# tuna2134/sbv2-api

Measured on AMD Instinct MI355X. Metric: audio_seconds_per_second, higher is better.
Workload: dtype bf16x3-split (decoder + flow convs: bf16 hi/lo MFMA, f32 accumulate/storage) + f16x3 (DeBERTa GEMMs, flow 1x1: f16 hi + scaled f16 lo per operand, 22 mantissa bits, f32 accumulate) + f32 (text side)

## Files before the change

include/sbv2_hip.h:

```cpp
#ifndef SBV2_HIP_H
#define SBV2_HIP_H

#include <stddef.h>
#include <stdint.h>

#ifdef __cplusplus
extern "C" {
#endif

typedef struct sbv2_bert sbv2_bert;
typedef struct sbv2_vits sbv2_vits;
typedef struct sbv2_pipeline sbv2_pipeline;

const char* sbv2_last_error(void);
int sbv2_device_count(void);

int sbv2_bert_create(const uint8_t* model, size_t model_len, int device, sbv2_bert** out);
void sbv2_bert_destroy(sbv2_bert* h);
int64_t sbv2_bert_hidden(const sbv2_bert* h);
int sbv2_bert_gemm_parts(const sbv2_bert* h);

int sbv2_bert_predict(sbv2_bert* h, const int64_t* token_ids, const int64_t* attention_mask, int64_t S, float* out);
int sbv2_bert_predict_batch(sbv2_bert* h, int64_t n, const int64_t* token_ids, const int64_t* attention_mask,
                            const int64_t* lens, float* out);
// ... 479 lines not shown
                                int64_t N, int poison, float* y, int64_t* stray);
int sbv2_debug_spline_inverse(int device, const float* params, const float* z, const uint8_t* mask, int64_t L, int64_t nbins, float tail, float inv_sqrt_f,
                              int poison, float* z_out, int64_t* stray);
int sbv2_debug_durations(int device, const float* sdp, const float* dp, const uint8_t* mask, int64_t L, float ratio, float length_scale, float* logw,
                         int32_t* dur, int64_t* stray);
int sbv2_debug_durations_rows(int device, const float* sdp, const float* dp, const uint8_t* mask, const int64_t* lens, int nutt, const float* ratio,
                              const float* length_scale, float* logw, int32_t* dur, int64_t* stray);
int sbv2_debug_affine_reverse(int device, const float* z, const float* m, const float* logs, const float* scale, const uint8_t* mask, int64_t L,
                              float* z_out, int64_t* stray);
int sbv2_debug_convflow_pre(int device, const float* z0, const float* w, const float* b, const float* cond, const uint8_t* mask, int64_t C, int64_t L,
                            float* y, int64_t* stray);
int sbv2_debug_noise_fill(int device, const int64_t* lens, int nutt, int kind, const int32_t* seg_utt, uint64_t seed, int stream_id, float scale,
                          int64_t rows, float* y, int64_t* stray);
int sbv2_debug_expand_frames(int device, const float* m_p, const float* logs_p, int64_t C, int64_t Lt, const int32_t* tok_of_frame, const int64_t* lens,
                             int nutt, const int32_t* seg_utt, uint64_t seed, float noise_scale, float* y, int64_t* stray);
int sbv2_debug_noise_fill_rows(int device, const int64_t* lens, int nutt, int kind, const uint64_t* seed, const int32_t* index, int stream_id,
                               const float* scale, int64_t rows, float* y, int64_t* stray);
int sbv2_debug_expand_frames_rows(int device, const float* m_p, const float* logs_p, int64_t C, int64_t Lt, const int32_t* tok_of_frame, const int64_t* lens,
                                  int nutt, const uint64_t* seed, const int32_t* index, const float* noise_scale, float* y, int64_t* stray);
int sbv2_debug_conv_post_tanh(int device, const float* x, const float* w, int64_t C, int64_t k, const int64_t* lens, int nutt, int64_t up, int cl,
                              float* pcm, int64_t* stray);
int sbv2_debug_linear_vec(int device, const float* W, const float* bias, int64_t M, int64_t K, const float* v, int64_t B, float* y);
int sbv2_debug_gather_rows(int device, const float* table, int64_t V, int64_t K, const int32_t* idx, int64_t B, float* y);
int sbv2_debug_text_embed(int device, const int32_t* phones, const int32_t* tones, const int32_t* langs, const int64_t* lens, int nutt, const float* emb,
                          int64_t nph, const float* tone_emb, int64_t ntone, const float* lang_emb, int64_t nlang, const float* bertproj,
                          const float* styleproj, float scale, int64_t H, float* y, int64_t* stray);
int sbv2_debug_add_segvec(int device, const float* x, const float* vec, int64_t C, const int64_t* lens, int nutt, int kind, int64_t div,
                          const uint8_t* tok_mask, int use_mask, int cl, float* y, int64_t* stray);
int sbv2_debug_plane_op(int device, int op, const float* x, int64_t C, int64_t L, const int32_t* map, int64_t a, int64_t b, float* y, uint8_t* mask_out,
                        int64_t* stray);
int sbv2_debug_stream_windows(int device, const float* z, int64_t C, int64_t L, const int32_t* table, int64_t W, int64_t nwin, const float* cond_vecs,
                              int64_t n_rows, int64_t cond_dim, float* z_out, uint8_t* mask_out, float* cond_out);
int sbv2_debug_copy_segments(int device, const float* src, int64_t nsrc, const int64_t* table, int nseg, float* dst, int64_t ndst);

#ifdef __cplusplus
}
#endif
#endif
```

sbv2-api_amd/_lib.py:

```python
import ctypes as C
import os

_HERE = os.path.dirname(os.path.abspath(__file__))
LIB_PATH = os.path.join(_HERE, "libsbv2_hip.so")

i64p = C.POINTER(C.c_int64)
f32p = C.POINTER(C.c_float)


class Sbv2Batch(C.Structure):
    _fields_ = [
        ("n", C.c_int64), ("t_lens", i64p), ("x_tst", i64p), ("tones", i64p), ("lang_ids", i64p), ("sids", i64p),
        ("style_vectors", f32p), ("bert", f32p),
        ("sdp_ratio", C.c_float), ("length_scale", C.c_float), ("noise_scale", C.c_float), ("noise_scale_w", C.c_float),
        ("noise_seed", C.c_uint64), ("forced_durations", i64p),
    ]


class Sbv2PcmFormat(C.Structure):
    _fields_ = [("sample_rate", C.c_int32), ("encoding", C.c_int32), ("normalize", C.c_int32), ("reserved", C.c_int32)]


class Sbv2Loudness(C.Structure):
    _fields_ = [("target_lufs", C.c_double), ("true_peak_max_dbtp", C.c_double)]
# ... 338 lines not shown
                                         i64p]),
    "sbv2_debug_gemm_bfs_ex": (C.c_int, [C.c_int, f32p, f32p, f32p, f32p, C.c_int64, C.c_int64, C.c_int64, C.c_int, C.c_int, C.c_int, C.c_int64, C.c_void_p,
                                         C.c_int64, C.c_float, C.c_float, C.c_int64, C.c_int64, C.c_int, f32p, f32p, f32p, i64p]),
    "sbv2_debug_linear_tokmajor": (C.c_int, [C.c_int, f32p, f32p, f32p, C.c_int64, C.c_int64, C.c_int64, C.c_int64, f32p, i64p]),
    "sbv2_debug_vits_attention": (C.c_int, [C.c_int, f32p, f32p, f32p, f32p, f32p, i64p, C.c_int, C.c_int64, C.c_int64, C.c_int64, C.c_int, C.c_int,
                                            C.c_int, f32p, i64p]),
    "sbv2_debug_deberta_attention": (C.c_int, [C.c_int, f32p, f32p, f32p, f32p, f32p, i64p, C.c_int, C.c_int64, C.c_int64, C.c_int64, C.c_int64,
                                               C.c_void_p, C.c_int64, C.c_int, C.c_int, f32p, i64p]),
    "sbv2_debug_layout": (C.c_int, [i64p, C.c_int, C.c_int, C.POINTER(C.c_int32), i64p]),
    "sbv2_debug_layernorm": (C.c_int, [C.c_int, f32p, f32p, f32p, C.c_float, C.c_int, f32p, C.c_void_p, f32p, f32p, C.c_int64, C.c_int64, C.c_int64, C.c_int,
                                       C.c_int, C.c_int, f32p, f32p, i64p]),
    "sbv2_debug_deberta_embed_ln": (C.c_int, [C.c_int, C.POINTER(C.c_int32), f32p, C.c_int64, C.c_int64, f32p, f32p, C.c_float, C.c_int64, C.c_int, f32p,
                                              i64p]),
    "sbv2_debug_spline_inverse": (C.c_int, [C.c_int, f32p, f32p, C.c_void_p, C.c_int64, C.c_int64, C.c_float, C.c_float, C.c_int, f32p, i64p]),
    "sbv2_debug_durations": (C.c_int, [C.c_int, f32p, f32p, C.c_void_p, C.c_int64, C.c_float, C.c_float, f32p, C.POINTER(C.c_int32), i64p]),
    "sbv2_debug_durations_rows": (C.c_int, [C.c_int, f32p, f32p, C.c_void_p, i64p, C.c_int, f32p, f32p, f32p, C.POINTER(C.c_int32), i64p]),
    "sbv2_debug_affine_reverse": (C.c_int, [C.c_int, f32p, f32p, f32p, f32p, C.c_void_p, C.c_int64, f32p, i64p]),
    "sbv2_debug_convflow_pre": (C.c_int, [C.c_int, f32p, f32p, f32p, f32p, C.c_void_p, C.c_int64, C.c_int64, f32p, i64p]),
    "sbv2_debug_noise_fill": (C.c_int, [C.c_int, i64p, C.c_int, C.c_int, C.POINTER(C.c_int32), C.c_uint64, C.c_int, C.c_float, C.c_int64, f32p, i64p]),
    "sbv2_debug_expand_frames": (C.c_int, [C.c_int, f32p, f32p, C.c_int64, C.c_int64, C.POINTER(C.c_int32), i64p, C.c_int, C.POINTER(C.c_int32), C.c_uint64,
                                           C.c_float, f32p, i64p]),
    "sbv2_debug_noise_fill_rows": (C.c_int, [C.c_int, i64p, C.c_int, C.c_int, C.POINTER(C.c_uint64), C.POINTER(C.c_int32), C.c_int, f32p, C.c_int64, f32p,
                                             i64p]),
    "sbv2_debug_expand_frames_rows": (C.c_int, [C.c_int, f32p, f32p, C.c_int64, C.c_int64, C.POINTER(C.c_int32), i64p, C.c_int, C.POINTER(C.c_uint64),
                                                C.POINTER(C.c_int32), f32p, f32p, i64p]),
    "sbv2_debug_conv_post_tanh": (C.c_int, [C.c_int, f32p, f32p, C.c_int64, C.c_int64, i64p, C.c_int, C.c_int64, C.c_int, f32p, i64p]),
    "sbv2_debug_linear_vec": (C.c_int, [C.c_int, f32p, f32p, C.c_int64, C.c_int64, f32p, C.c_int64, f32p]),
    "sbv2_debug_gather_rows": (C.c_int, [C.c_int, f32p, C.c_int64, C.c_int64, C.POINTER(C.c_int32), C.c_int64, f32p]),
    "sbv2_debug_text_embed": (C.c_int, [C.c_int, C.POINTER(C.c_int32), C.POINTER(C.c_int32), C.POINTER(C.c_int32), i64p, C.c_int, f32p, C.c_int64, f32p,
                                        C.c_int64, f32p, C.c_int64, f32p, f32p, C.c_float, C.c_int64, f32p, i64p]),
    "sbv2_debug_add_segvec": (C.c_int, [C.c_int, f32p, f32p, C.c_int64, i64p, C.c_int, C.c_int, C.c_int64, C.c_void_p, C.c_int, C.c_int, f32p, i64p]),
    "sbv2_debug_plane_op": (C.c_int, [C.c_int, C.c_int, f32p, C.c_int64, C.c_int64, C.POINTER(C.c_int32), C.c_int64, C.c_int64, f32p, C.c_void_p, i64p]),
    "sbv2_debug_copy_segments": (C.c_int, [C.c_int, f32p, C.c_int64, i64p, C.c_int, f32p, C.c_int64]),
}

_lib = None


class Sbv2Error(RuntimeError):
    """Mirror of sbv2_core::error::Error::OtherError (crates/sbv2_core/src/error.rs:29-30)."""


def lib():
    global _lib
    if _lib is None:
        if not os.path.exists(LIB_PATH):
            raise Sbv2Error(f"{LIB_PATH} is missing: build it with __graft_entry__.build() (there is no CPU fallback)")
        l = C.CDLL(LIB_PATH)
        for name, (res, args) in SYMBOLS.items():
            fn = getattr(l, name)
            fn.restype = res
            fn.argtypes = args
        _lib = l
    return _lib


def check(rc):
    if rc != 0:
        raise Sbv2Error(lib().sbv2_last_error().decode(errors="replace"))
```

sbv2-api_amd/csrc/common.h:

```cpp
#pragma once
#include <hip/hip_runtime.h>

#include <atomic>

#include <cstdint>
#include <cstdio>
#include <map>
#include <memory>
#include <stdexcept>
#include <exception>
#include <string>
#include <vector>

namespace sbv2 {

void set_last_error(const std::string& msg);

struct Error : std::runtime_error {
    using std::runtime_error::runtime_error;
};

#define HIP_CHECK(expr)                                                                          \
    do {                                                                                         \
        hipError_t _e = (expr);                                                                  \
// ... 417 lines not shown
    int shift0 = 0, shift_step = 1;
    float* Y = nullptr;
    int ldy = 0;
    float* Ykm = nullptr;
    int ldykm = 0;
    const float* Rkm = nullptr;
    int ldrkm = 0;
    SplitClPlanes Ys;
    float ys_slope = 1.0f;
    const float* bias = nullptr;
    const float* R = nullptr;
    int ldr = 0;
    float beta = 1.0f;
    int accumulate = 0;
    const unsigned char* mask = nullptr;
    int mask_shift = -1;
    int out_stride = 1, phase_rows = 0;
    int phase_off[kMaxPhases] = {0};
    int phase_group = 1;
    int phase_tap0[kMaxPhases] = {0};
    double prof_flops = 0.0;
};
int64_t clx_grid_workgroups(const ConvClxParams& p);
bool conv_clx_usable(const ConvClxParams& p);
int set_clx(int on);
int set_upx(int on);
int set_resbranch(int on);
int set_respair_clx(int on);
bool ksplit_enabled();
int set_ksplit(int on);
bool clx_wanted(int64_t tiles, int64_t min_tiles);
void launch_conv_clx(const ConvClxParams& p, hipStream_t stream);

struct ResPairParams {
    const float* X = nullptr;
    float* Y = nullptr;
    const void* W1 = nullptr;
    const void* W2 = nullptr;
    const void* W1p = nullptr;
    const void* W2p = nullptr;
    const void* W1x = nullptr;
    const void* W2x = nullptr;
    const float* b1 = nullptr;
    const float* b2 = nullptr;
    int C = 0, N = 0, k = 1, dil = 1, split = 1, f16 = 0;
    float slope = 0.1f, beta = 1.0f;
    int accumulate = 0;
    const unsigned char* mask = nullptr;
    int mask_div = 1;
    int mask_shift = -1;
    int alias_x2 = 1;
    int nt_store = 0;
};
void launch_respair_cl(const ResPairParams& p, hipStream_t stream);
bool respair_clx_usable(const ResPairParams& p);
void launch_respair_clx(const ResPairParams& p, hipStream_t stream);
bool respair_x16_usable(const ResPairParams& p);
void launch_respair_x16(const ResPairParams& p, hipStream_t stream);
enum class BranchKernel { resbranch, clx_steps, respair_x16, respair_clx, respair_cl, conv_cl_steps };
BranchKernel respair_default(const ResPairParams& p);
void launch_respair(const ResPairParams& p, BranchKernel kernel, hipStream_t stream);

constexpr int kResBranchSteps = 3;
constexpr int kResBranchMargin = 6;
struct ResBranchParams {
    const float* X = nullptr;
// ... 17 lines not shown
```

sbv2-api_amd/csrc/models.h:

```cpp
#pragma once
#include "common.h"
#include "flac_encode.h"
#include "limiter.h"
#include "marks.h"
#include "ops.h"
#include "pcm_format.h"
#include "stream_output.h"

#include <memory>

namespace sbv2 {

struct ClConv {
    void* w = nullptr;
    void* wxp = nullptr;
    void* wx = nullptr;
    void* wp = nullptr;
    float* bias = nullptr;
    int M = 0, K = 0, k = 1, nmt = 0, tm = 1, parts = 0;
};

struct PackedConv {
    float* w = nullptr;
    float* bias = nullptr;
// ... 67 lines not shown
    float* upload(const float* host, size_t n);
    float* tensor(const std::string& name);
    float* tensor(const std::string& name, std::initializer_list<int64_t> dims);
    void expect(const PackedConv& c, const std::string& prefix, int cout, int cin, int k) const;
    PackedConv conv(const std::string& prefix, bool bias = true);
    PackedConv conv_cat(const std::vector<std::string>& prefixes);
    PackedConv linear(const std::string& prefix);
    PackedUpsample upsample(const std::string& prefix, int stride, int padding);
    size_t bytes() const { return bytes_; }
    const Blob& blob() const { return blob_; }

  private:
    const Blob& blob_;
    int cl_parts_ = 0, bfs_parts_ = 0;
    std::vector<void*> allocs_;
    size_t bytes_ = 0;
};

void conv_plain(const PackedConv& w, Plane x, Plane y, int dil, int pad_l, const unsigned char* mask, int mask_div, hipStream_t s,
                int act = ACT_NONE, float pre_slope = 1.0f, const Plane* res = nullptr, float alpha = 1.0f, float beta = 1.0f,
                int accumulate = 0);
void conv_bfs(const PackedConv& w, const SplitPlanes& xs, const Plane* y, const SplitPlanes* ys, const unsigned char* mask, int mask_div,
              hipStream_t s, int act = ACT_NONE, const Plane* res = nullptr, float alpha = 1.0f, float beta = 1.0f, int y_rows = -1, int ys_row0 = 0,
              const BfsSplitK* sk = nullptr);
bool conv_km_to_cl(const PackedConv& w, Plane x, float* y, int ldy, int dil, int pad_l, const unsigned char* mask, int mask_div,
                   hipStream_t s);
bool conv_cl_to_km(const PackedConv& w, const float* x, int ldx, Plane y, int dil, int pad_l, const unsigned char* mask, int mask_div,
                   hipStream_t s, float pre_slope, const Plane* res);
void linear_tokmajor(const PackedConv& w, Plane x, float* y, int ldy, hipStream_t s);

int default_bert_bfs_parts();
bool flash_parts_enabled();
int set_flash_parts(int on);
bool sdp_all();
int set_sdp_all(int on);

constexpr int kTextGap = 16;
constexpr int kFrameGap = 4;
struct AttnPlan {
    int ng = 0, maxT = 0, lds = 0;
    AttnGroup* d_ag = nullptr;
    GemmGroup* d_st = nullptr;
    GemmGroup* d_pv = nullptr;
    float* S = nullptr;
    float* PW = nullptr;
    double flops = 0;
};
AttnPlan make_attn_plan(const SegLayout& lay, int H, int heads, int ld, int window, Arena& ar, hipStream_t stream, bool scores);
void grouped_gemm(const float* A, int lda, const float* B, int ldb, float* C, int ldc, const GemmGroup* grp, int ng, int maxM, int maxN,
                  float alpha, double flops, hipStream_t s);
struct FlashChoice {
    bool kv_parts = false;
    int pipelined = 1;
};
FlashChoice flash_choice(const AttnPlan& pl, int SP, bool split_attn, int dk);

enum DebertaAttnMode {
    kDbAuto = -1,
    kDbUnfused = 0,
    kDbShort = 1,
    kDbMid = 2,
    kDbLong = 3,
    kDbNoLong = 4,
};
struct DebertaAttnPlan {
    int span = 0, maxT = 0, lds = 0;
// ... 314 lines not shown
```

sbv2-api_amd/csrc/vits.cpp:

```cpp
#include <algorithm>
#include <cmath>
#include <cstring>
#include <memory>

#include <atomic>
#include "models.h"

namespace sbv2 {

static std::atomic<int> g_flash_parts{1};
bool flash_parts_enabled() { return g_flash_parts.load(std::memory_order_relaxed) != 0; }
static int flash_parts_mode() { return g_flash_parts.load(std::memory_order_relaxed); }
int set_flash_parts(int on) { return g_flash_parts.exchange(on); }

static std::atomic<int> g_sdp_all{0};
bool sdp_all() { return g_sdp_all.load(std::memory_order_relaxed) != 0; }
int set_sdp_all(int on) { return g_sdp_all.exchange(on != 0); }

AttnPlan make_attn_plan(const SegLayout& lay, int H, int heads, int ld, int window, Arena& ar, hipStream_t stream, bool scores) {
    AttnPlan pl;
    const int dk = H / heads;
    pl.ng = lay.n * heads;
    pl.maxT = lay.max_len();
    pl.lds = round_up(pl.maxT, 4);
    std::vector<AttnGroup> ag(pl.ng);
    std::vector<GemmGroup> st(pl.ng), pv(pl.ng);
    int64_t s_off = 0, w_off = 0;
    for (int u = 0; u < lay.n; ++u)
        for (int h = 0; h < heads; ++h) {
            const int gi = u * heads + h;
            const int T = lay.len[u];
            AttnGroup& a = ag[gi];
            a.qk_off = (int64_t)h * dk * ld + lay.start[u];
            a.s_off = s_off;
            a.aux_off = w_off;
            a.aux2_off = 0;
            a.T = T;
            a.lds = pl.lds;
            a.col0 = lay.start[u];
            a.head = h;
            st[gi] = GemmGroup{a.qk_off, a.qk_off, s_off, 0, T, T, dk, T};
            pv[gi] = GemmGroup{(int64_t)lay.start[u] * H + h * dk, s_off, a.qk_off, 0, dk, T, T, T};
            pl.flops += 2.0 * (double)T * T * dk;
            s_off += (int64_t)T * pl.lds;
            w_off += (int64_t)(2 * window + 1) * pl.lds;
        }
// ... 280 lines not shown
    if (it == traces_.end()) return false;
    const TraceEntry& t = it->second;
    if (utt < 0 || utt >= t.lay->n) return false;
    HIP_CHECK(hipSetDevice(device_));
    rows = t.p.C;
    cols = t.lay->len[utt] * t.div;
    out.resize((size_t)rows * cols);
    HIP_CHECK(hipStreamSynchronize(stream_));
    HIP_CHECK(hipMemcpy2D(out.data(), sizeof(float) * cols, t.p.p + (size_t)t.lay->start[utt] * t.div, sizeof(float) * t.p.ld,
                          sizeof(float) * cols, rows, hipMemcpyDeviceToHost));
    return true;
}

void VitsModel::run_encoder(const Encoder& e, Plane x, const SegLayout& lay, const float* spk_vec, Arena& ar) {
    const int H = x.C, heads = cfg_.heads, dk = H / heads, N = lay.L;
    const Arena::Mark mk = ar.mark();
    static const bool fused = !(getenv("SBV2_ATTN") && std::string(getenv("SBV2_ATTN")) == "unfused");
    static const bool attn_f32 = getenv("SBV2_ATTN") && std::string(getenv("SBV2_ATTN")) == "f32";
    const bool split_attn = !attn_f32 && e.layers[0].ffn1.cl.parts == 2 && (H / heads) % 16 == 0;
    const AttnPlan pl = make_attn_plan(lay, H, heads, x.ld, cfg_.window, ar, stream_, !fused);
    Plane QKV = ar.plane(3 * H, N);
    Plane Q = QKV.rows(0, H), K = QKV.rows(H, H), ctx = ar.plane(H, N), Y = ar.plane(H, N);
    SBV2_REQUIRE(Q.ld == x.ld, "plane pitch mismatch");
    Plane F = ar.plane(e.layers[0].ffn1.cout, N);
    constexpr bool cl_ffn = true;
    const PackedConv& f1 = e.layers[0].ffn1;
    const PackedConv& f2 = e.layers[0].ffn2;
    float* Fcl = (cl_ffn && f1.cl.parts && f2.cl.parts && f1.k >= 3 && f2.k >= 3 && (f1.cout & 15) == 0) ? ar.array<float>((size_t)N * f1.cout) : nullptr;
    float* VT = fused ? nullptr : ar.array<float>((size_t)N * H);
    Plane Vp = QKV.rows(2 * H, H);
    fill_zero(ctx.p, sizeof(float) * (size_t)H * ctx.ld, stream_);
    const float qscale = 1.0f / std::sqrt((float)dk);
    const int SP = !fused ? 0 : (e.layers[0].attn.qkv.bfs.f16 ? kPartsF16x3 : e.layers[0].attn.qkv.bfs.parts);
    SplitPlanes Xs, Cs, QKVs;
    if (SP) {
        Xs = alloc_split(ar, SP, H, N);
        Cs = alloc_split(ar, SP, H, N);
        split_planes(x, Xs, stream_);
    }
    const FlashChoice fc = flash_choice(pl, SP, split_attn, dk);
    const bool kv_parts = fc.kv_parts;
    if (kv_parts) QKVs = alloc_split(ar, 2, 3 * H, N);
    const bool clx_ffn = Fcl && f1.cl.parts == 2 && f2.cl.parts == 2 && f1.k == 5 && f2.k == 5 && (H & 63) == 0 && (f1.cout & 63) == 0 &&
                         clx_wanted((int64_t)(N / 256) * (H / 64), 192);
    SplitClPlanes XsC, FsC;
    if (clx_ffn) {
        XsC = make_split_cl(ar.alloc(split_cl_bytes(H, N)), H, N, stream_);
        FsC = make_split_cl(ar.alloc(split_cl_bytes(f1.cout, N)), f1.cout, N, stream_);
    }
    for (size_t i = 0; i < e.layers.size(); ++i) {
        const EncLayer& L = e.layers[i];
        if ((int)i == cfg_.cond_layer_idx && spk_vec) {
            add_segvec(x, spk_vec, H, lay.d_seg_of, 1, lay.d_mask, stream_);
            if (SP) split_planes(x, Xs, stream_);
        }
        if (fused) {
            if (SP && kv_parts) conv_bfs(L.attn.qkv, Xs, &QKV, &QKVs, nullptr, 1, stream_, ACT_NONE, nullptr, 1.0f, 1.0f, H, H);
            else if (SP) conv_bfs(L.attn.qkv, Xs, &QKV, nullptr, nullptr, 1, stream_);
            else conv_plain(L.attn.qkv, x, QKV, 1, 0, nullptr, 1, stream_);
            if (kv_parts)
                vits_flash_attention_parts(pl.d_ag, pl.ng, pl.maxT, Q.p, Q.ld, QKVs, H, 2 * H, ctx.p, ctx.ld, dk, L.attn.erk, L.attn.erv, cfg_.window,
                                           qscale, stream_, fc.pipelined);
            else
                vits_flash_attention(pl.d_ag, pl.ng, pl.maxT, Q.p, K.p, Vp.p, Q.ld, ctx.p, ctx.ld, dk, L.attn.erk, L.attn.erv, cfg_.window, qscale,
                                     split_attn, stream_);
        } else {
            conv_plain(L.attn.q, x, Q, 1, 0, nullptr, 1, stream_);
            conv_plain(L.attn.k, x, K, 1, 0, nullptr, 1, stream_);
            linear_tokmajor(L.attn.v, x, VT, H, stream_);
            grouped_gemm(K.p, K.ld, Q.p, Q.ld, pl.S, pl.lds, pl.d_st, pl.ng, pl.maxT, pl.maxT, qscale, pl.flops, stream_);
            vits_softmax(pl.d_ag, pl.ng, pl.maxT, pl.S, Q.p, Q.ld, dk, L.attn.erk, cfg_.window, qscale, pl.PW, stream_);
            grouped_gemm(VT, H, pl.S, pl.lds, ctx.p, ctx.ld, pl.d_pv, pl.ng, dk, pl.maxT, 1.0f, pl.flops, stream_);
            vits_relv_add(pl.d_ag, pl.ng, pl.maxT, ctx.p, ctx.ld, dk, L.attn.erv, cfg_.window, pl.PW, stream_);
        }
        if (SP) {
            split_planes(ctx, Cs, stream_);
            conv_bfs(L.attn.o, Cs, &Y, nullptr, nullptr, 1, stream_, ACT_NONE, &x);
        } else {
            conv_plain(L.attn.o, ctx, Y, 1, 0, nullptr, 1, stream_, ACT_NONE, 1.0f, &x);
        }
        layernorm_ch(Y, x, L.n1g, L.n1b, 1e-5f, ACT_NONE, nullptr, 0, lay.d_mask, stream_);
        const int k = L.ffn1.k;
        const int Fc = L.ffn1.cout;
        if (clx_ffn) {
            split_cl_km(x, 1.0f, XsC, stream_);
            ConvClxParams p1;
            p1.X = XsC;
            p1.W = L.ffn1.cl.wx;
            p1.nmt = L.ffn1.cl.nmt;
            p1.M = Fc;
            p1.N = N;
            p1.K = H;
            p1.ntaps = k;
            p1.shift0 = -(k - 1) / 2;
            p1.shift_step = 1;
            p1.Ys = FsC;
            p1.ys_slope = 0.0f;
            p1.bias = L.ffn1.bias;
            p1.mask = lay.d_mask;
            p1.mask_shift = 0;
            launch_conv_clx(p1, stream_);
            ConvClxParams p2;
            p2.X = FsC;
            p2.W = L.ffn2.cl.wx;
            p2.nmt = L.ffn2.cl.nmt;
            p2.M = H;
            p2.N = N;
            p2.K = Fc;
            p2.ntaps = k;
            p2.shift0 = -(k - 1) / 2;
            p2.shift_step = 1;
            p2.Ykm = Y.p;
            p2.ldykm = Y.ld;
            p2.Rkm = x.p;
            p2.ldrkm = x.ld;
            p2.bias = L.ffn2.bias;
            p2.mask = lay.d_mask;
            p2.mask_shift = 0;
            launch_conv_clx(p2, stream_);
        } else if (Fcl && conv_km_to_cl(L.ffn1, x, Fcl, Fc, 1, (k - 1) / 2, lay.d_mask, 1, stream_)) {
            SBV2_REQUIRE(conv_cl_to_km(L.ffn2, Fcl, Fc, Y, 1, (k - 1) / 2, lay.d_mask, 1, stream_, 0.0f, &x), "FFN: conv_2 has no matrix-core path");
        } else {
            conv_plain(L.ffn1, x, F, 1, (k - 1) / 2, lay.d_mask, 1, stream_, ACT_RELU);
            conv_plain(L.ffn2, F, Y, 1, (k - 1) / 2, lay.d_mask, 1, stream_, ACT_NONE, 1.0f, &x);
        }
        layernorm_ch(Y, x, L.n2g, L.n2b, 1e-5f, ACT_NONE, nullptr, 0, lay.d_mask, stream_, (SP && i + 1 < e.layers.size()) ? &Xs : nullptr);
    }
    ar.rewind(mk);
}

void VitsModel::run_dds(const DDS& d, Plane x, const SegLayout& lay, Arena& ar, int shape_L) {
    const Arena::Mark mk = ar.mark();
    Plane a = ar.plane(x.C, x.L), b = ar.plane(x.C, x.L);
    int dil = 1;
    for (size_t i = 0; i < d.pw.size(); ++i) {
        dds_dw_ln_gelu(x, a, d.sep_w[i], d.sep_b[i], dil, d.n1g[i], d.n1b[i], lay.d_mask, stream_, shape_L);
        conv_plain(d.pw[i], a, b, 1, 0, nullptr, 1, stream_);
        layernorm_ch(b, x, d.n2g[i], d.n2b[i], 1e-5f, ACT_GELU, x.p, x.ld, lay.d_mask, stream_, nullptr, shape_L);
        dil *= cfg_.sdp_kernel;
    }
    ar.rewind(mk);
}

void VitsModel::run_decoder(Arena& ar, Plane z, const SegLayout& fl, const float* cond_vec) {
    const int n = fl.n;
    const int Lf = fl.L;
    Plane cur = ar.plane(cfg_.up_initial, Lf);
    conv_plain(dec_pre_, z, cur, 1, dec_pre_.k / 2, fl.d_mask, 1, stream_);
    add_segvec(cur, cond_vec, cfg_.up_initial, fl.d_seg_of, 1, fl.d_mask, stream_);
    trace("dec_pre", cur, fl, 1);
    int U = 1;
    const int nk = (int)cfg_.res_kernels.size();
    for (size_t si = 0; si < stages_.size(); ++si) {
        const Stage& st = stages_[si];
        U *= st.rate;
        const int Lo = Lf * U;
        Plane XS = ar.plane(st.ch, Lo);
        const Arena::Mark mk = ar.mark();
        Plane XU = ar.plane(st.ch, Lo), T1 = ar.plane(st.ch, Lo), YA = ar.plane(st.ch, Lo), YB = ar.plane(st.ch, Lo);
// ... 672 lines not shown
```

Before: 4833.

## Fuse flow encoder attention-out projection with layernorm and FFN tail with next QKV

```diff
diff --git a/include/sbv2_hip.h b/include/sbv2_hip.h
--- a/include/sbv2_hip.h
+++ b/include/sbv2_hip.h
@@ -535,6 +535,14 @@
 int sbv2_debug_stream_windows(int device, const float* z, int64_t C, int64_t L, const int32_t* table, int64_t W, int64_t nwin, const float* cond_vecs,
                               int64_t n_rows, int64_t cond_dim, float* z_out, uint8_t* mask_out, float* cond_out);
 int sbv2_debug_copy_segments(int device, const float* src, int64_t nsrc, const int64_t* table, int nseg, float* dst, int64_t ndst);
+int sbv2_debug_set_flow_cols(int mode);
+int sbv2_debug_set_flow_cols_block(int nct);
+int sbv2_debug_flow_attn_tail(int device, const float* ctx, const float* x, const float* w, const float* bias, const float* gamma, const float* beta, float eps,
+                              const uint8_t* mask, int64_t N, int64_t ld, int want_parts, int64_t iters, float* x_out, uint16_t* parts, float* ms,
+                              int64_t* stray);
+int sbv2_debug_flow_ffn_tail_qkv(int device, const float* y, const float* gamma, const float* beta, float eps, const uint8_t* mask, const float* spk, int64_t nseg,
+                                 const int32_t* seg_of, const float* w, const float* bias, int64_t N, int64_t ld, int kv_parts, int64_t iters, float* x_out,
+                                 float* qkv, uint16_t* kv, float* ms, int64_t* stray);
 
 #ifdef __cplusplus
 }
diff --git a/sbv2-api_amd/_lib.py b/sbv2-api_amd/_lib.py
--- a/sbv2-api_amd/_lib.py
+++ b/sbv2-api_amd/_lib.py
@@ -394,6 +394,12 @@
     "sbv2_debug_add_segvec": (C.c_int, [C.c_int, f32p, f32p, C.c_int64, i64p, C.c_int, C.c_int, C.c_int64, C.c_void_p, C.c_int, C.c_int, f32p, i64p]),
     "sbv2_debug_plane_op": (C.c_int, [C.c_int, C.c_int, f32p, C.c_int64, C.c_int64, C.POINTER(C.c_int32), C.c_int64, C.c_int64, f32p, C.c_void_p, i64p]),
     "sbv2_debug_copy_segments": (C.c_int, [C.c_int, f32p, C.c_int64, i64p, C.c_int, f32p, C.c_int64]),
+    "sbv2_debug_set_flow_cols": (C.c_int, [C.c_int]),
+    "sbv2_debug_set_flow_cols_block": (C.c_int, [C.c_int]),
+    "sbv2_debug_flow_attn_tail": (C.c_int, [C.c_int, f32p, f32p, f32p, f32p, f32p, f32p, C.c_float, C.c_void_p, C.c_int64, C.c_int64, C.c_int, C.c_int64,
+                                            f32p, C.c_void_p, f32p, i64p]),
+    "sbv2_debug_flow_ffn_tail_qkv": (C.c_int, [C.c_int, f32p, f32p, f32p, C.c_float, C.c_void_p, f32p, C.c_int64, C.POINTER(C.c_int32), f32p, f32p, C.c_int64,
+                                               C.c_int64, C.c_int, C.c_int64, f32p, f32p, C.c_void_p, f32p, i64p]),
 }
 
 _lib = None
diff --git a/sbv2-api_amd/csrc/common.h b/sbv2-api_amd/csrc/common.h
--- a/sbv2-api_amd/csrc/common.h
+++ b/sbv2-api_amd/csrc/common.h
@@ -473,6 +473,48 @@
 bool clx_wanted(int64_t tiles, int64_t min_tiles);
 void launch_conv_clx(const ConvClxParams& p, hipStream_t stream);
 
+constexpr int kFlowColsH = 192;
+struct FlowAttnTailParams {
+    const float* ctx = nullptr;
+    int ldc = 0;
+    float* x = nullptr;
+    int ldx = 0;
+    const void* w = nullptr;
+    int nmt = 0;
+    const float* bias = nullptr;
+    const float* gamma = nullptr;
+    const float* beta = nullptr;
+    float eps = 1e-5f;
+    const unsigned char* mask = nullptr;
+    int N = 0;
+    SplitClPlanes xs;
+    unsigned long long* sat = nullptr;
+};
+struct FlowFfnTailParams {
+    const float* Y = nullptr;
+    int ldy = 0;
+    float* x = nullptr;
+    int ldx = 0;
+    const float* gamma = nullptr;
+    const float* beta = nullptr;
+    float eps = 1e-5f;
+    const unsigned char* mask = nullptr;
+    const float* spk = nullptr;
+    int spk_ld = 0;
+    const int* seg_of = nullptr;
+    const void* w = nullptr;
+    int nmt = 0;
+    const float* bias = nullptr;
+    float* qkv = nullptr;
+    int ldq = 0;
+    SplitPlanes kv;
+    int N = 0;
+    unsigned long long* sat = nullptr;
+};
+void launch_flow_attn_tail(const FlowAttnTailParams& p, hipStream_t stream);
+void launch_flow_ffn_tail_qkv(const FlowFfnTailParams& p, hipStream_t stream);
+int set_flow_cols_block(int nct);
+
 struct ResPairParams {
     const float* X = nullptr;
     float* Y = nullptr;
diff --git a/sbv2-api_amd/csrc/flow_cols.hip b/sbv2-api_amd/csrc/flow_cols.hip
--- /dev/null
+++ b/sbv2-api_amd/csrc/flow_cols.hip
@@ -0,0 +1,387 @@
+#include <atomic>
+
+#include "common.h"
+#include "device_prims.h"
+
+namespace sbv2 {
+
+namespace {
+
+constexpr int kH = kFlowColsH;
+constexpr int kNCH = kH / 16;
+constexpr int kBStr = 2 * kH + 16;
+constexpr int kFStr = kH + 4;
+static_assert(kH == 192, "three 32-row tiles per wave, two waves per column tile");
+
+template <int NCT>
+struct Shape {
+    static constexpr int NB = 32 * NCT, NQ = NB / 4, T = 128 * NCT, NW = 2 * NCT;
+    static constexpr int BPART = NB * kBStr;
+    static constexpr int IMG = 2 * BPART;
+    static constexpr int RED = 2 * 2 * NB * (int)sizeof(float);
+    static constexpr int TILES = NW * 32 * 36 * (int)sizeof(float);
+    static_assert(NB * kFStr * (int)sizeof(float) <= IMG, "the result image fits the operand image");
+    static_assert(2 * 16 * NQ * 16 <= TILES, "the partial sums fit the transpose tiles");
+};
+
+__device__ __forceinline__ void split_f16(float v, _Float16& h, _Float16& l, unsigned& nclamp, bool count) {
+    const float c = (v != v || fabsf(v) == __builtin_inff()) ? v : fminf(fmaxf(v, -65504.f), 65504.f);
+    nclamp += (count && c != v && v == v) ? 1u : 0u;
+    h = (_Float16)c;
+    l = (_Float16)((c - (float)h) * kF16LoScale);
+}
+
+template <int NCT>
+__device__ __forceinline__ void stage_operand(char* img, const f32x4v (&v)[3][4], int cq, int kq0, int n0, int N, unsigned& nclamp) {
+    using S = Shape<NCT>;
+#pragma unroll
+    for (int i = 0; i < 3; ++i)
+#pragma unroll
+        for (int e = 0; e < 4; ++e) {
+            f16x4 h, l;
+            const bool count = n0 + 4 * cq + e < N;
+#pragma unroll
+            for (int j = 0; j < 4; ++j) {
+                _Float16 hh, ll;
+                split_f16(v[i][j][e], hh, ll, nclamp, count);
+                h[j] = hh;
+                l[j] = ll;
+            }
+            char* dst = img + (4 * cq + e) * kBStr + (kq0 + 16 * i) * 8;
+            *reinterpret_cast<f16x4*>(dst) = h;
+            *reinterpret_cast<f16x4*>(dst + S::BPART) = l;
+        }
+}
+
+template <int NCT>
+__device__ __forceinline__ void product(const char* img, const void* w, int nmt, int mt0, int ct, int lane, f32x16 (&acc)[3], f32x16 (&accx)[3]) {
+    using S = Shape<NCT>;
+    const char* wl = static_cast<const char*>(w) + lane * 16;
+    const char* bl = img + (ct * 32 + (lane & 31)) * kBStr + (lane >> 5) * 16;
+    constexpr int kAhead = 3, NBUF = kAhead + 1;
+    f16x8 a[NBUF][3][2];
+    auto load = [&](int c, f16x8 (&f)[3][2]) {
+#pragma unroll
+        for (int i = 0; i < 3; ++i)
+#pragma unroll
+            for (int pp = 0; pp < 2; ++pp) f[i][pp] = *reinterpret_cast<const f16x8*>(wl + ((int64_t)(c * nmt + mt0 + i) * 2 + pp) * 1024);
+    };
+#pragma unroll
+    for (int i = 0; i < 3; ++i)
+#pragma unroll
+        for (int r = 0; r < 16; ++r) acc[i][r] = accx[i][r] = 0.f;
+#pragma unroll
+    for (int c = 0; c < kAhead; ++c) load(c, a[c]);
+#pragma unroll
+    for (int c = 0; c < kNCH; ++c) {
+        if (c + kAhead < kNCH) load(c + kAhead, a[(c + kAhead) % NBUF]);
+        __builtin_amdgcn_sched_barrier(0);
+        const f16x8 bh = *reinterpret_cast<const f16x8*>(bl + c * 32), bo = *reinterpret_cast<const f16x8*>(bl + S::BPART + c * 32);
+        const f16x8(&f)[3][2] = a[c % NBUF];
+#pragma unroll
+        for (int i = 0; i < 3; ++i) accx[i] = mfma32(f[i][1], bh, accx[i]);
+#pragma unroll
+        for (int i = 0; i < 3; ++i) accx[i] = mfma32(f[i][0], bo, accx[i]);
+#pragma unroll
+        for (int i = 0; i < 3; ++i) acc[i] = mfma32(f[i][0], bh, acc[i]);
+    }
+}
+
+template <int NCT>
+__global__ __launch_bounds__(128 * NCT) __attribute__((amdgpu_waves_per_eu(2))) void k_flow_attn_tail(const FlowAttnTailParams p) {
+    using S = Shape<NCT>;
+    extern __shared__ __attribute__((aligned(16))) char smem[];
+    char* img = smem;
+    float* fimg = reinterpret_cast<float*>(smem);
+    float* red = reinterpret_cast<float*>(smem + S::IMG);
+    const int tid = threadIdx.x, lane = tid & 63, wave = tid >> 6;
+    const int n0 = blockIdx.x * S::NB, N = p.N;
+    const int cq = tid % S::NQ, kq0 = tid / S::NQ;
+    const int nq = n0 + 4 * cq, nql = nq < N ? nq : 0;
+    unsigned nclamp = 0;
+    {
+        f32x4v v[3][4];
+#pragma unroll
+        for (int i = 0; i < 3; ++i)
+#pragma unroll
+            for (int j = 0; j < 4; ++j) v[i][j] = *reinterpret_cast<const f32x4v*>(p.ctx + (int64_t)(4 * (kq0 + 16 * i) + j) * p.ldc + nql);
+        stage_operand<NCT>(img, v, cq, kq0, n0, N, nclamp);
+    }
+    if (p.sat && nclamp) atomicAdd(p.sat, (unsigned long long)nclamp);
+    __syncthreads();
+    const int mh = wave & 1, ct = wave >> 1, lh = lane >> 5;
+    const int col = ct * 32 + (lane & 31), n = n0 + col, nl = n < N ? n : 0;
+    f32x16 acc[3], accx[3];
+    product<NCT>(img, p.w, p.nmt, 3 * mh, ct, lane, acc, accx);
+    float s = 0.f;
+#pragma unroll
+    for (int i = 0; i < 3; ++i)
+#pragma unroll
+        for (int r = 0; r < 16; ++r) {
+            const int m = (3 * mh + i) * 32 + (r & 3) + 8 * (r >> 2) + 4 * lh;
+            float y = acc[i][r] + accx[i][r] * (1.0f / kF16LoScale) + p.bias[m];
+            y += p.x[(int64_t)m * p.ldx + nl];
+            acc[i][r] = y;
+            s += y;
+        }
+    s += __shfl_xor(s, 32);
+    if (lh == 0) red[mh * S::NB + col] = s;
+    __syncthreads();
+    const float mean = (red[col] + red[S::NB + col]) / (float)kH;
+    float q = 0.f;
+#pragma unroll
+    for (int i = 0; i < 3; ++i)
+#pragma unroll
+        for (int r = 0; r < 16; ++r) {
+            const float d = acc[i][r] - mean;
+            q += d * d;
+        }
+    q += __shfl_xor(q, 32);
+    if (lh == 0) red[(2 + mh) * S::NB + col] = q;
+    __syncthreads();
+    const float var = red[2 * S::NB + col] + red[3 * S::NB + col];
+    const float rstd = 1.0f / sqrtf(var / kH + p.eps);
+    const bool keep = n < N && (!p.mask || p.mask[nl]);
+#pragma unroll
+    for (int i = 0; i < 3; ++i)
+#pragma unroll
+        for (int g = 0; g < 4; ++g) {
+            const int m = (3 * mh + i) * 32 + 8 * g + 4 * lh;
+            const f32x4v ga = *reinterpret_cast<const f32x4v*>(p.gamma + m), be = *reinterpret_cast<const f32x4v*>(p.beta + m);
+            f32x4v y;
+#pragma unroll
+            for (int e = 0; e < 4; ++e) {
+                const float t = (acc[i][4 * g + e] - mean) * rstd * ga[e] + be[e];
+                y[e] = keep ? t : 0.f;
+            }
+            *reinterpret_cast<f32x4v*>(fimg + col * kFStr + m) = y;
+        }
+    __syncthreads();
+#pragma unroll
+    for (int i = 0; i < 3; ++i) {
+        const int k4 = 4 * (kq0 + 16 * i);
+        f32x4v r[4];
+#pragma unroll
+        for (int e = 0; e < 4; ++e) r[e] = *reinterpret_cast<const f32x4v*>(fimg + (4 * cq + e) * kFStr + k4);
+#pragma unroll
+        for (int j = 0; j < 4; ++j) {
+            float* dst = p.x + (int64_t)(k4 + j) * p.ldx + nq;
+            if (nq + 4 <= N) {
+                *reinterpret_cast<f32x4v*>(dst) = f32x4v{r[0][j], r[1][j], r[2][j], r[3][j]};
+            } else {
+#pragma unroll
+                for (int e = 0; e < 4; ++e)
+                    if (nq + e < N) dst[e] = r[e][j];
+            }
+        }
+    }
+    if (p.xs.p) {
+        const int64_t plane = (int64_t)(p.xs.front + p.xs.N + p.xs.back) * 32;
+#pragma unroll
+        for (int i = 0; i < 3; ++i) {
+            const int u = tid + S::T * i, pc = u % S::NB, ch = u / S::NB;
+            if (n0 + pc >= N) continue;
+            bf16x8 h[2], l[2];
+#pragma unroll
+            for (int g = 0; g < 4; ++g) {
+                const f32x4v v = *reinterpret_cast<const f32x4v*>(fimg + pc * kFStr + ch * 16 + 4 * g);
+#pragma unroll
+                for (int e = 0; e < 4; ++e) {
+                    const __bf16 hh = (__bf16)v[e];
+                    h[g >> 1][(g & 1) * 4 + e] = hh;
+                    l[g >> 1][(g & 1) * 4 + e] = (__bf16)(v[e] - (float)hh);
+                }
+            }
+            char* dst = static_cast<char*>(p.xs.p) + ((int64_t)ch * 2) * plane + ((int64_t)p.xs.front + n0 + pc) * 32;
+            *reinterpret_cast<bf16x8*>(dst) = h[0];
+            *reinterpret_cast<bf16x8*>(dst + 16) = h[1];
+            *reinterpret_cast<bf16x8*>(dst + plane) = l[0];
+            *reinterpret_cast<bf16x8*>(dst + plane + 16) = l[1];
+        }
+    }
+}
+
+template <int NCT>
+__global__ __launch_bounds__(128 * NCT) __attribute__((amdgpu_waves_per_eu(2))) void k_flow_ffn_tail_qkv(const FlowFfnTailParams p) {
+    using S = Shape<NCT>;
+    typedef f32x4v red_t[S::NQ];
+    extern __shared__ __attribute__((aligned(16))) char smem[];
+    char* img = smem;
+    const int tid = threadIdx.x, lane = tid & 63, wave = tid >> 6;
+    const int n0 = blockIdx.x * S::NB, N = p.N;
+    const int cq = tid % S::NQ, kq0 = tid / S::NQ;
+    const int nq = n0 + 4 * cq, nql = nq < N ? nq : 0;
+    unsigned nclamp = 0;
+    {
+        red_t* red = reinterpret_cast<red_t*>(smem + S::IMG);
+        f32x4v v[3][4];
+        f32x4v s = {0.f, 0.f, 0.f, 0.f};
+#pragma unroll
+        for (int i = 0; i < 3; ++i)
+#pragma unroll
+            for (int j = 0; j < 4; ++j) {
+                v[i][j] = *reinterpret_cast<const f32x4v*>(p.Y + (int64_t)(4 * (kq0 + 16 * i) + j) * p.ldy + nql);
+                s += v[i][j];
+            }
+        auto reduce = [&](red_t* r, f32x4v part) {
+            r[kq0][cq] = part;
+            __syncthreads();
+            f32x4v t = r[0][cq];
+#pragma unroll
+            for (int g = 1; g < 16; ++g) t += r[g][cq];
+            return t;
+        };
+        const f32x4v mean = reduce(red, s) / (float)kH;
+        f32x4v q = {0.f, 0.f, 0.f, 0.f};
+#pragma unroll
+        for (int i = 0; i < 3; ++i)
+#pragma unroll
+            for (int j = 0; j < 4; ++j) {
+                const f32x4v d = v[i][j] - mean;
+                q += d * d;
+            }
+        const f32x4v var = reduce(red + 16, q);
+        f32x4v rstd;
+        bool keep[4];
+        int sg[4];
+#pragma unroll
+        for (int e = 0; e < 4; ++e) {
+            rstd[e] = 1.0f / sqrtf(var[e] / kH + p.eps);
+            const int ne = nq + e < N ? nq + e : 0;
+            keep[e] = nq + e < N && (!p.mask || p.mask[ne]);
+            sg[e] = p.spk ? p.seg_of[ne] : -1;
+        }
+#pragma unroll
+        for (int i = 0; i < 3; ++i) {
+            const int k4 = 4 * (kq0 + 16 * i);
+            const f32x4v ga = *reinterpret_cast<const f32x4v*>(p.gamma + k4), be = *reinterpret_cast<const f32x4v*>(p.beta + k4);
+#pragma unroll
+            for (int j = 0; j < 4; ++j) {
+                f32x4v y;
+#pragma unroll
+                for (int e = 0; e < 4; ++e) {
+                    const float t = (v[i][j][e] - mean[e]) * rstd[e] * ga[j] + be[j];
+                    y[e] = keep[e] ? t : 0.f;
+                    if (p.spk) y[e] = (sg[e] >= 0 && keep[e]) ? y[e] + p.spk[(int64_t)sg[e] * p.spk_ld + k4 + j] : 0.f;
+                }
+                v[i][j] = y;
+                float* dst = p.x + (int64_t)(k4 + j) * p.ldx + nq;
+                if (nq + 4 <= N) {
+                    *reinterpret_cast<f32x4v*>(dst) = y;
+                } else {
+#pragma unroll
+                    for (int e = 0; e < 4; ++e)
+                        if (nq + e < N) dst[e] = y[e];
+                }
+            }
+        }
+        stage_operand<NCT>(img, v, cq, kq0, n0, N, nclamp);
+    }
+    if (p.sat && nclamp) atomicAdd(p.sat, (unsigned long long)nclamp);
+    __syncthreads();
+    const int mh = wave & 1, ct = wave >> 1, lh = lane >> 5, lcol = lane & 31;
+    const int lrow = lane >> 3, c4 = (lane & 7) * 4;
+    float* tile = reinterpret_cast<float*>(smem + S::IMG) + wave * (32 * 36);
+    const int nc = n0 + ct * 32 + c4;
+#pragma unroll 1
+    for (int pass = 0; pass < 3; ++pass) {
+        f32x16 acc[3], accx[3];
+        const int mt0 = 6 * pass + 3 * mh;
+        product<NCT>(img, p.w, p.nmt, mt0, ct, lane, acc, accx);
+        const bool parts = p.kv.p && pass > 0;
+#pragma unroll
+        for (int i = 0; i < 3; ++i) {
+#pragma unroll
+            for (int r = 0; r < 16; ++r) tile[((r & 3) + 8 * (r >> 2) + 4 * lh) * 36 + lcol] = acc[i][r] + accx[i][r] * (1.0f / kF16LoScale);
+#pragma unroll
+            for (int ps = 0; ps < 4; ++ps) {
+                const f32x4v av = *reinterpret_cast<const f32x4v*>(tile + (ps * 8 + lrow) * 36 + c4);
+                const int m = (mt0 + i) * 32 + ps * 8 + lrow;
+                const float b = p.bias[m];
+                float v[4];
+#pragma unroll
+                for (int e = 0; e < 4; ++e) v[e] = av[e] + b;
+                if (nc >= N) continue;
+                if (!parts) {
+                    float* dst = p.qkv + (int64_t)m * p.ldq + nc;
+                    if (nc + 4 <= N) {
+                        *reinterpret_cast<f32x4v*>(dst) = f32x4v{v[0], v[1], v[2], v[3]};
+                    } else {
+#pragma unroll
+                        for (int e = 0; e < 4; ++e)
+                            if (nc + e < N) dst[e] = v[e];
+                    }
+                } else {
+                    bf16x4 h, l;
+#pragma unroll
+                    for (int e = 0; e < 4; ++e) {
+                        h[e] = (__bf16)v[e];
+                        l[e] = (__bf16)(v[e] - (float)h[e]);
+                    }
+                    __bf16* dst = static_cast<__bf16*>(p.kv.p) + (int64_t)m * p.kv.ld + nc;
+                    if (nc + 4 <= N) {
+                        *reinterpret_cast<bf16x4*>(dst) = h;
+                        *reinterpret_cast<bf16x4*>(dst + p.kv.pstride) = l;
+                    } else {
+#pragma unroll
+                        for (int e = 0; e < 4; ++e)
+                            if (nc + e < N) {
+                                dst[e] = h[e];
+                                dst[p.kv.pstride + e] = l[e];
+                            }
+                    }
+                }
+            }
+        }
+    }
+}
+
+std::atomic<int> g_block{2};
+
+template <class P>
+void check_common(const P& p, int rows, const char* what) {
+    SBV2_REQUIRE(p.w && p.bias && p.gamma && p.beta && p.N >= 1 && p.nmt * 32 >= rows, what);
+}
+
+template <int NCT, class K, class P>
+void launch_cfg(K kern, const P& p, size_t lds, hipStream_t stream, std::atomic<uint64_t>& done) {
+    allow_full_lds(reinterpret_cast<const void*>(kern), done);
+    hipLaunchKernelGGL(kern, dim3((p.N + 32 * NCT - 1) / (32 * NCT)), dim3(128 * NCT), lds, stream, p);
+    HIP_CHECK(hipGetLastError());
+}
+
+}
+
+int set_flow_cols_block(int nct) {
+    if (nct != 1 && nct != 2 && nct != 4) return -1;
+    return g_block.exchange(nct);
+}
+
+void launch_flow_attn_tail(const FlowAttnTailParams& p, hipStream_t stream) {
+    check_common(p, kH, "flow_attn_tail: missing operand");
+    SBV2_REQUIRE(p.ctx && p.x && (p.ldc & 3) == 0 && (p.ldx & 3) == 0 && p.ldc >= round_up(p.N, 4) && p.ldx >= round_up(p.N, 4), "flow_attn_tail: plane pitch");
+    SBV2_REQUIRE(!p.xs.p || (p.xs.C == kH && p.xs.N == p.N), "flow_attn_tail: parts shape");
+    static std::atomic<uint64_t> done[3];
+    switch (g_block.load(std::memory_order_relaxed)) {
+        case 1: launch_cfg<1>(k_flow_attn_tail<1>, p, Shape<1>::IMG + Shape<1>::RED, stream, done[0]); break;
+        case 4: launch_cfg<4>(k_flow_attn_tail<4>, p, Shape<4>::IMG + Shape<4>::RED, stream, done[2]); break;
+        default: launch_cfg<2>(k_flow_attn_tail<2>, p, Shape<2>::IMG + Shape<2>::RED, stream, done[1]); break;
+    }
+}
+
+void launch_flow_ffn_tail_qkv(const FlowFfnTailParams& p, hipStream_t stream) {
+    check_common(p, 3 * kH, "flow_ffn_tail_qkv: missing operand");
+    SBV2_REQUIRE(p.Y && p.x && p.qkv && (p.ldy & 3) == 0 && (p.ldx & 3) == 0 && (p.ldq & 3) == 0 && p.ldy >= round_up(p.N, 4) && p.ldx >= round_up(p.N, 4) &&
+                     p.ldq >= round_up(p.N, 4),
+                 "flow_ffn_tail_qkv: plane pitch");
+    SBV2_REQUIRE(!p.kv.p || (p.kv.parts == 2 && !p.kv.f16 && p.kv.C == 3 * kH && (p.kv.ld & 3) == 0 && p.kv.ld >= round_up(p.N, 4)), "flow_ffn_tail_qkv: parts shape");
+    SBV2_REQUIRE(!p.spk || (p.seg_of && p.spk_ld >= kH), "flow_ffn_tail_qkv: speaker vector without the segment table");
+    static std::atomic<uint64_t> done[3];
+    switch (g_block.load(std::memory_order_relaxed)) {
+        case 1: launch_cfg<1>(k_flow_ffn_tail_qkv<1>, p, Shape<1>::IMG + Shape<1>::TILES, stream, done[0]); break;
+        case 4: launch_cfg<4>(k_flow_ffn_tail_qkv<4>, p, Shape<4>::IMG + Shape<4>::TILES, stream, done[2]); break;
+        default: launch_cfg<2>(k_flow_ffn_tail_qkv<2>, p, Shape<2>::IMG + Shape<2>::TILES, stream, done[1]); break;
+    }
+}
+
+}
diff --git a/sbv2-api_amd/csrc/models.h b/sbv2-api_amd/csrc/models.h
--- a/sbv2-api_amd/csrc/models.h
+++ b/sbv2-api_amd/csrc/models.h
@@ -123,6 +123,7 @@
 int default_bert_bfs_parts();
 bool flash_parts_enabled();
 int set_flash_parts(int on);
+int set_flow_cols(int mode);
 bool sdp_all();
 int set_sdp_all(int on);
 
diff --git a/sbv2-api_amd/csrc/vits.cpp b/sbv2-api_amd/csrc/vits.cpp
--- a/sbv2-api_amd/csrc/vits.cpp
+++ b/sbv2-api_amd/csrc/vits.cpp
@@ -12,6 +12,9 @@
 bool flash_parts_enabled() { return g_flash_parts.load(std::memory_order_relaxed) != 0; }
 static int flash_parts_mode() { return g_flash_parts.load(std::memory_order_relaxed); }
 int set_flash_parts(int on) { return g_flash_parts.exchange(on); }
+
+static std::atomic<int> g_flow_cols{1};
+int set_flow_cols(int mode) { return (mode < 0 || mode > 2) ? -1 : g_flow_cols.exchange(mode); }
 
 static std::atomic<int> g_sdp_all{0};
 bool sdp_all() { return g_sdp_all.load(std::memory_order_relaxed) != 0; }
@@ -358,10 +361,13 @@
     fill_zero(ctx.p, sizeof(float) * (size_t)H * ctx.ld, stream_);
     const float qscale = 1.0f / std::sqrt((float)dk);
     const int SP = !fused ? 0 : (e.layers[0].attn.qkv.bfs.f16 ? kPartsF16x3 : e.layers[0].attn.qkv.bfs.parts);
+    const int cols_mode = g_flow_cols.load(std::memory_order_relaxed);
+    const bool cols = fused && H == kFlowColsH && SP == kPartsF16x3 && e.layers[0].attn.o.bfs.f16 && e.layers[0].attn.o.bfs.M == H &&
+                      e.layers[0].attn.qkv.bfs.M == 3 * H && (cols_mode == 2 || (cols_mode == 1 && clx_wanted((int64_t)(N / 256) * (H / 64), 192)));
     SplitPlanes Xs, Cs, QKVs;
     if (SP) {
         Xs = alloc_split(ar, SP, H, N);
-        Cs = alloc_split(ar, SP, H, N);
+        if (!cols) Cs = alloc_split(ar, SP, H, N);
         split_planes(x, Xs, stream_);
     }
     const FlashChoice fc = flash_choice(pl, SP, split_attn, dk);
@@ -376,14 +382,17 @@
     }
     for (size_t i = 0; i < e.layers.size(); ++i) {
         const EncLayer& L = e.layers[i];
-        if ((int)i == cfg_.cond_layer_idx && spk_vec) {
+        const bool qkv_done = cols && i > 0;
+        if ((int)i == cfg_.cond_layer_idx && spk_vec && !qkv_done) {
             add_segvec(x, spk_vec, H, lay.d_seg_of, 1, lay.d_mask, stream_);
             if (SP) split_planes(x, Xs, stream_);
         }
         if (fused) {
-            if (SP && kv_parts) conv_bfs(L.attn.qkv, Xs, &QKV, &QKVs, nullptr, 1, stream_, ACT_NONE, nullptr, 1.0f, 1.0f, H, H);
-            else if (SP) conv_bfs(L.attn.qkv, Xs, &QKV, nullptr, nullptr, 1, stream_);
-            else conv_plain(L.attn.qkv, x, QKV, 1, 0, nullptr, 1, stream_);
+            if (!qkv_done) {
+                if (SP && kv_parts) conv_bfs(L.attn.qkv, Xs, &QKV, &QKVs, nullptr, 1, stream_, ACT_NONE, nullptr, 1.0f, 1.0f, H, H);
+                else if (SP) conv_bfs(L.attn.qkv, Xs, &QKV, nullptr, nullptr, 1, stream_);
+                else conv_plain(L.attn.qkv, x, QKV, 1, 0, nullptr, 1, stream_);
+            }
             if (kv_parts)
                 vits_flash_attention_parts(pl.d_ag, pl.ng, pl.maxT, Q.p, Q.ld, QKVs, H, 2 * H, ctx.p, ctx.ld, dk, L.attn.erk, L.attn.erv, cfg_.window,
                                            qscale, stream_, fc.pipelined);
@@ -399,17 +408,35 @@
             grouped_gemm(VT, H, pl.S, pl.lds, ctx.p, ctx.ld, pl.d_pv, pl.ng, dk, pl.maxT, 1.0f, pl.flops, stream_);
             vits_relv_add(pl.d_ag, pl.ng, pl.maxT, ctx.p, ctx.ld, dk, L.attn.erv, cfg_.window, pl.PW, stream_);
         }
-        if (SP) {
-            split_planes(ctx, Cs, stream_);
-            conv_bfs(L.attn.o, Cs, &Y, nullptr, nullptr, 1, stream_, ACT_NONE, &x);
+        if (cols) {
+            FlowAttnTailParams t;
+            t.ctx = ctx.p;
+            t.ldc = ctx.ld;
+            t.x = x.p;
+            t.ldx = x.ld;
+            t.w = L.attn.o.bfs.w;
+            t.nmt = L.attn.o.bfs.nmt;
+            t.bias = L.attn.o.bias;
+            t.gamma = L.n1g;
+            t.beta = L.n1b;
+            t.mask = lay.d_mask;
+            t.N = N;
+            if (clx_ffn) t.xs = XsC;
+            t.sat = Xs.sat;
+            launch_flow_attn_tail(t, stream_);
         } else {
-            conv_plain(L.attn.o, ctx, Y, 1, 0, nullptr, 1, stream_, ACT_NONE, 1.0f, &x);
-        }
-        layernorm_ch(Y, x, L.n1g, L.n1b, 1e-5f, ACT_NONE, nullptr, 0, lay.d_mask, stream_);
+            if (SP) {
+                split_planes(ctx, Cs, stream_);
+                conv_bfs(L.attn.o, Cs, &Y, nullptr, nullptr, 1, stream_, ACT_NONE, &x);
+            } else {
+                conv_plain(L.attn.o, ctx, Y, 1, 0, nullptr, 1, stream_, ACT_NONE, 1.0f, &x);
+            }
+            layernorm_ch(Y, x, L.n1g, L.n1b, 1e-5f, ACT_NONE, nullptr, 0, lay.d_mask, stream_);
+        }
         const int k = L.ffn1.k;
         const int Fc = L.ffn1.cout;
         if (clx_ffn) {
-            split_cl_km(x, 1.0f, XsC, stream_);
+            if (!cols) split_cl_km(x, 1.0f, XsC, stream_);
             ConvClxParams p1;
             p1.X = XsC;
             p1.W = L.ffn1.cl.wx;
@@ -450,7 +477,33 @@
             conv_plain(L.ffn1, x, F, 1, (k - 1) / 2, lay.d_mask, 1, stream_, ACT_RELU);
             conv_plain(L.ffn2, F, Y, 1, (k - 1) / 2, lay.d_mask, 1, stream_, ACT_NONE, 1.0f, &x);
         }
-        layernorm_ch(Y, x, L.n2g, L.n2b, 1e-5f, ACT_NONE, nullptr, 0, lay.d_mask, stream_, (SP && i + 1 < e.layers.size()) ? &Xs : nullptr);
+        if (cols && i + 1 < e.layers.size()) {
+            const EncLayer& Ln = e.layers[i + 1];
+            FlowFfnTailParams t;
+            t.Y = Y.p;
+            t.ldy = Y.ld;
+            t.x = x.p;
+            t.ldx = x.ld;
+            t.gamma = L.n2g;
+            t.beta = L.n2b;
+            t.mask = lay.d_mask;
+            if ((int)i + 1 == cfg_.cond_layer_idx && spk_vec) {
+                t.spk = spk_vec;
+                t.spk_ld = H;
+                t.seg_of = lay.d_seg_of;
+            }
+            t.w = Ln.attn.qkv.bfs.w;
+            t.nmt = Ln.attn.qkv.bfs.nmt;
+            t.bias = Ln.attn.qkv.bias;
+            t.qkv = QKV.p;
+            t.ldq = QKV.ld;
+            if (kv_parts) t.kv = QKVs;
+            t.N = N;
+            t.sat = Xs.sat;
+            launch_flow_ffn_tail_qkv(t, stream_);
+        } else {
+            layernorm_ch(Y, x, L.n2g, L.n2b, 1e-5f, ACT_NONE, nullptr, 0, lay.d_mask, stream_, (SP && !cols && i + 1 < e.layers.size()) ? &Xs : nullptr);
+        }
     }
     ar.rewind(mk);
 }
```

Result: no change. 4851, median of 2 (+0.4%).
